# lucidrains/voicebox-pytorch

Hardware: AMD Instinct MI355X
Metric: mel-frames/sec train-step (fwd+bwd+allreduce+clip+Adam) (higher is better)
Workload: dtype f16/bf16 (fp16 forward operands, bf16 backward operands, fp32 accumulate/master); 1 GPU; VoiceBox dim 512 depth 12 heads 16 unconditional, 8x1024 frames per GPU, train; global_batch=8, seq_len=1024, parallelism=dp1

## Files before the change

voicebox-pytorch_amd/csrc/ops.hip:

```cpp
#include "common.hpp"
#include "reduce_roles.hpp"
#include <stdlib.h>

namespace {

VBX_DEV void unpack8_bf16(const uint4 p, float v[8]) {
  const unsigned w[4] = {p.x, p.y, p.z, p.w};
#pragma unroll
  for (int i = 0; i < 4; i++) {
    v[2 * i] = bf16_to_f32((u16)(w[i] & 0xffff));
    v[2 * i + 1] = bf16_to_f32((u16)(w[i] >> 16));
  }
}
VBX_DEV void unpack8_f16(const uint4 p, float v[8]) {
  const unsigned w[4] = {p.x, p.y, p.z, p.w};
#pragma unroll
  for (int i = 0; i < 4; i++) {
    v[2 * i] = f16_to_f32((u16)(w[i] & 0xffff));
    v[2 * i + 1] = f16_to_f32((u16)(w[i] >> 16));
  }
}
VBX_DEV uint4 pack8_h(const float v[8]) {
  return make_uint4(pack_f16x2_sat(v[0], v[1]), pack_f16x2_sat(v[2], v[3]), pack_f16x2_sat(v[4], v[5]), pack_f16x2_sat(v[6], v[7]));
}
// ... 135 lines not shown
    int i0, i1;
    float lam;
    interp_src(n, N, T, i0, i1, lam);
    const float g = bf16_to_f32(demb[row * ld + e]);
    const long id0 = dropped ? null_id : ids[(long)b * T + i0], id1 = dropped ? null_id : ids[(long)b * T + i1];
    if (T == N) {
      atomicAdd(gtable + id0 * E + e, g);
    } else {
      atomicAdd(gtable + id0 * E + e, (1.0f - lam) * g);
      atomicAdd(gtable + id1 * E + e, lam * g);
    }
  }
}

constexpr int CT = 64;
template <int MODE, int KS>
__global__ __launch_bounds__(256) void convpos_fwd_kernel(const float* __restrict__ e, const float* __restrict__ w,
                                                          const float* __restrict__ bias, const uint8_t* __restrict__ mask,
                                                          const float* __restrict__ dxs, float* __restrict__ out, int N,
                                                          int R, int D) {
  extern __shared__ float tile[];
  constexpr int ks = KS;
  const int half = ks / 2;
  const int n0 = blockIdx.x * CT, dbase = blockIdx.y * 64, b = blockIdx.z;
  const int dl = threadIdx.x & 63, ng = threadIdx.x >> 6;
  const int d = dbase + dl;
  const int rows = CT + ks - 1;
  for (int r = ng; r < rows; r += 4) {
    const int n = n0 + r - half;
    float v = 0.f;
    if (n >= 0 && n < N && d < D && (!mask || mask[(long)b * N + n])) v = e[((long)b * N + n) * D + d];
    tile[r * 64 + dl] = v;
  }
  __syncthreads();
  if (d >= D) return;
  float wr[KS];
#pragma unroll
  for (int k = 0; k < ks; k++) wr[k] = w[(long)d * ks + k];
  const float bb = bias[d];
  const int Np = N + R;
  for (int i = 0; i < 16; i++) {
    const int nl = ng * 16 + i, n = n0 + nl;
    if (n >= N) break;
    float acc = bb;
#pragma unroll
    for (int k = 0; k < ks; k++) acc += wr[k] * tile[(nl + k) * 64 + dl];
    const bool m = !mask || mask[(long)b * N + n];
    if (MODE == 0 || MODE == 2) {
      const float ev = e[((long)b * N + n) * D + d];
      out[((long)b * Np + R + n) * D + d] = ev + (m ? (MODE == 2 ? gelu_erf_libm(acc) : gelu_erf(acc)) : 0.f);
    } else {
      const float g = dxs[((long)b * Np + R + n) * D + d];
      out[((long)b * N + n) * D + d] = m ? g * gelu_erf_grad(acc) : 0.f;
    }
  }
}

template <int KS>
__global__ __launch_bounds__(256) void convpos_fwd_segs_kernel(const float* __restrict__ e, const float* __restrict__ w,
                                                               const float* __restrict__ bias, const float* __restrict__ reg,
                                                               const int* __restrict__ seg_start, const int* __restrict__ seg_klen,
                                                               const int* __restrict__ tile_seg, float* __restrict__ out, int R, int D) {
  extern __shared__ float tile[];
  constexpr int ks = KS;
  const int half = ks / 2;
  const int r0 = blockIdx.x * CT, dbase = blockIdx.y * 64;
  const int dl = threadIdx.x & 63, ng = threadIdx.x >> 6;
  const int d = dbase + dl;
// ... 87 lines not shown
    reinterpret_cast<float4*>(dx)[i] = a;
    if (dxb) reinterpret_cast<uint2*>(dxb)[i] = make_uint2(pack_bf16x2(a.x, a.y), pack_bf16x2(a.z, a.w));
  }
}

__global__ void regs_fill_kernel(const float* __restrict__ reg, float* __restrict__ xs, int B, int Np, int R, int D) {
  const long total = (long)B * R * D;
  for (long i = blockIdx.x * (long)blockDim.x + threadIdx.x; i < total; i += (long)gridDim.x * blockDim.x) {
    const int b = (int)(i / ((long)R * D));
    const long rd = i - (long)b * R * D;
    xs[(long)b * Np * D + rd] = reg[rd];
  }
}

template <int KS>
__global__ __launch_bounds__(256) void convpos_bwd_kernel(const float* __restrict__ e, const float* __restrict__ w,
                                                          const uint8_t* __restrict__ mask, const float* __restrict__ dxs,
                                                          const float* __restrict__ dpre, float* __restrict__ de,
                                                          u16* __restrict__ deb, float* __restrict__ wpart, int N, int R,
                                                          int D) {
  extern __shared__ float sm[];
  constexpr int ks = KS;
  static_assert(KS <= 31, "wacc holds the taps in [0, KS) and the bias gradient in [31]");
  const int half = ks / 2;
  const int rows = CT + ks - 1;
  float* te = sm;
  float* tp = sm + rows * 64;
  const int n0 = blockIdx.x * CT, dbase = blockIdx.y * 64, b = blockIdx.z;
  const int dl = threadIdx.x & 63, ng = threadIdx.x >> 6;
  const int d = dbase + dl;
  for (int r = ng; r < rows; r += 4) {
    const int n = n0 + r - half;
    float ve = 0.f, vp = 0.f;
    if (n >= 0 && n < N && d < D) {
      if (!mask || mask[(long)b * N + n]) ve = e[((long)b * N + n) * D + d];
      vp = dpre[((long)b * N + n) * D + d];
    }
    te[r * 64 + dl] = ve;
    tp[r * 64 + dl] = vp;
  }
  __syncthreads();
  float wr[KS], wacc[32];
#pragma unroll
  for (int k = 0; k < 32; k++) wacc[k] = 0.f;
  if (d < D) {
#pragma unroll
    for (int k = 0; k < ks; k++) wr[k] = w[(long)d * ks + k];
    const int Np = N + R;
    for (int i = 0; i < 16; i++) {
      const int nl = ng * 16 + i, n = n0 + nl;
      if (n >= N) break;
      float acc = 0.f;
#pragma unroll
      for (int k = 0; k < ks; k++) acc += wr[k] * tp[(nl + 2 * half - k) * 64 + dl];
      const bool m = !mask || mask[(long)b * N + n];
      const float o = dxs[((long)b * Np + R + n) * D + d] + (m ? acc : 0.f);
      de[((long)b * N + n) * D + d] = o;
      if (deb) deb[((long)b * N + n) * D + d] = f32_to_bf16(o);
      const float dp = tp[(nl + half) * 64 + dl];
#pragma unroll
      for (int k = 0; k < ks; k++) wacc[k] += dp * te[(nl + k) * 64 + dl];
      wacc[31] += dp;
    }
  }
  __syncthreads();
  float* red = sm;
#pragma unroll
  for (int k = 0; k < 32; k++) red[(ng * 64 + dl) * 33 + k] = wacc[k];
  __syncthreads();
  const long chunk = (long)b * gridDim.x + blockIdx.x;
  for (int idx = threadIdx.x; idx < 64 * 32; idx += 256) {
    const int c = idx >> 5, k = idx & 31;
    if (dbase + c < D) {
      const float s = red[(0 * 64 + c) * 33 + k] + red[(1 * 64 + c) * 33 + k] + red[(2 * 64 + c) * 33 + k] +
                      red[(3 * 64 + c) * 33 + k];
      wpart[(chunk * D + dbase + c) * 64 + (k == 31 ? 63 : k)] = s;
    }
  }
}

__global__ void conv_wgrad_finalize_kernel(const float* __restrict__ wpart, int chunks, int D, int ks, float* __restrict__ dw,
                                           float* __restrict__ db) {
  const int idx = blockIdx.x * blockDim.x + threadIdx.x;
  if (idx >= D * 64) return;
  const int d = idx >> 6, k = idx & 63;
  if (k >= ks && k != 63) return;
  float s = 0.f;
  int c = 0;
  for (; c + 4 <= chunks; c += 4) {
    float v[4];
// ... 566 lines not shown
        const float4 v = *reinterpret_cast<const float4*>(reinterpret_cast<const float*>(in) + r * ld + c0);
        acc[0] += v.x; acc[1] += v.y; acc[2] += v.z; acc[3] += v.w;
      }
    }
  }
#pragma unroll
  for (int i = 0; i < W; i++) red[rl][cgi][i] = acc[i];
  __syncthreads();
  if (rl == 0 && c0 < C) {
#pragma unroll
    for (int i = 0; i < W; i++)
      scratch[(long)slab * C + c0 + i] = red[0][cgi][i] + red[1][cgi][i] + red[2][cgi][i] + red[3][cgi][i];
  }
}
__global__ __launch_bounds__(1024) void multi_reduce_kernel(vbx_mr_jobs jobs) {
  __shared__ float red[16][64];
  int j = 0;
#pragma unroll
  for (int i = 1; i < VBX_MR_MAX; i++)
    if (i < jobs.n && (int)blockIdx.x >= jobs.job[i].block0) j = i;
  const vbx_mr_job jb = jobs.job[j];
  mr_role(jb, blockIdx.x - jb.block0, red);
}
__global__ __launch_bounds__(1024) void layer_reduce_kernel(vbx_skr_jobs sj, vbx_mr_jobs mj, int skr_blocks) {
  __shared__ float red[16][64];
  if ((int)blockIdx.x < skr_blocks) {
    int j = 0;
#pragma unroll
    for (int i = 1; i < VBX_SKR_MAX; i++)
      if (i < sj.n && (int)blockIdx.x >= sj.job[i].block0) j = i;
    const vbx_skr_job jb = sj.job[j];
    (void)skr_role(jb, ((long)(blockIdx.x - jb.block0) * 1024 + threadIdx.x) * 4);
    return;
  }
  const int bx = blockIdx.x - skr_blocks;
  int j = 0;
#pragma unroll
  for (int i = 1; i < VBX_MR_MAX; i++)
    if (i < mj.n && bx >= mj.job[i].block0) j = i;
  const vbx_mr_job jb = mj.job[j];
// ... 583 lines not shown

#define VBX_CONV_KS_SWITCH(ks, CALL)                                                                                      \
  switch (ks) {                                                                                                           \
    case 1: CALL(1); break;   case 3: CALL(3); break;   case 5: CALL(5); break;   case 7: CALL(7); break;                 \
    case 9: CALL(9); break;   case 11: CALL(11); break; case 13: CALL(13); break; case 15: CALL(15); break;               \
    case 17: CALL(17); break; case 19: CALL(19); break; case 21: CALL(21); break; case 23: CALL(23); break;               \
    case 25: CALL(25); break; case 27: CALL(27); break; case 29: CALL(29); break; default: CALL(31); break;               \
  }
static inline bool conv_ks_ok(int ks) { return ks >= 1 && ks <= 31 && (ks & 1); }

static int convpos_fwd_impl(const float* e, const float* w, const float* bias, const uint8_t* mask, const float* reg, float* xs, int B,
                            int N, int R, int D, int ksize, bool libm, void* stream) {
  VBX_REQUIRE(e && w && bias && xs, "vbx_convpos_fwd: null pointer");
  VBX_REQUIRE(conv_ks_ok(ksize), "vbx_convpos_fwd: conv_pos_embed_kernel_size must be odd and <= 31 (got %d)", ksize);
  VBX_REQUIRE(R == 0 || reg, "vbx_convpos_fwd: register tokens missing");
  dim3 grid(cdiv(N, CT), cdiv(D, 64), B);
#define VBX_CALL(KS)                                                                                                           \
  if (libm)                                                                                                                    \
    hipLaunchKernelGGL((convpos_fwd_kernel<2, KS>), grid, dim3(256), (CT + KS - 1) * 64 * sizeof(float), ST, e, w, bias, mask, \
                       (const float*)nullptr, xs, N, R, D);                                                                    \
  else                                                                                                                         \
    hipLaunchKernelGGL((convpos_fwd_kernel<0, KS>), grid, dim3(256), (CT + KS - 1) * 64 * sizeof(float), ST, e, w, bias, mask, \
                       (const float*)nullptr, xs, N, R, D)
  VBX_CONV_KS_SWITCH(ksize, VBX_CALL)
#undef VBX_CALL
  VBX_LAUNCH_CHECK();
  if (R > 0) {
    hipLaunchKernelGGL(regs_fill_kernel, dim3(grid_for((long)B * R * D)), dim3(256), 0, ST, reg, xs, B, N + R, R, D);
    VBX_LAUNCH_CHECK();
  }
  return 0;
}

extern "C" int vbx_convpos_fwd(const float* e, const float* w, const float* bias, const uint8_t* mask, const float* reg,
                               float* xs, int B, int N, int R, int D, int ksize, void* stream) {
  return convpos_fwd_impl(e, w, bias, mask, reg, xs, B, N, R, D, ksize, false, stream);
}
extern "C" int vbx_convpos_fwd_libm(const float* e, const float* w, const float* bias, const uint8_t* mask, const float* reg,
                                    float* xs, int B, int N, int R, int D, int ksize, void* stream) {
  return convpos_fwd_impl(e, w, bias, mask, reg, xs, B, N, R, D, ksize, true, stream);
}

extern "C" int vbx_convpos_fwd_segs(const float* e, const float* w, const float* bias, const float* reg, const int* seg_start,
                                    const int* seg_klen, const int* tile_seg, float* xs, int Mp, int R, int D, int ksize, void* stream) {
  VBX_REQUIRE(e && w && bias && xs && seg_start && seg_klen && tile_seg, "vbx_convpos_fwd_segs: null pointer");
// ... 45 lines not shown
  VBX_REQUIRE(dxs && dx && B > 0 && N > 0 && R >= 0 && D % 4 == 0, "vbx_stack_input_bwd: bad args");
  hipLaunchKernelGGL(stack_rows_kernel, dim3(grid_for((long)B * N * D / 4)), dim3(256), 0, ST, dxs, dx, B, N, R, D, 0);
  VBX_LAUNCH_CHECK();
  if (R > 0 && dreg) {
    hipLaunchKernelGGL(dreg_kernel, dim3(cdiv((long)R * D, 256)), dim3(256), 0, ST, dxs, dreg, B, N + R, R, D);
    VBX_LAUNCH_CHECK();
  }
  return 0;
}

extern "C" int vbx_convpos_bwd_chunks(int B, int N) { return B * cdiv(N, CT); }

extern "C" int vbx_convpos_bwd(const float* e, const float* w, const float* bias, const uint8_t* mask, const float* dxs,
                               float* dpre_tmp, float* de, void* de_bf16, float* wpart, float* dreg, int B, int N, int R,
                               int D, int ksize, void* stream) {
  VBX_REQUIRE(e && w && bias && dxs && dpre_tmp && de && wpart, "vbx_convpos_bwd: null pointer");
  VBX_REQUIRE(conv_ks_ok(ksize), "vbx_convpos_bwd: conv_pos_embed_kernel_size must be odd and <= 31 (got %d)", ksize);
  dim3 grid(cdiv(N, CT), cdiv(D, 64), B);
  const int rows = CT + ksize - 1;
#define VBX_CALL(KS)                                                                                                            \
  hipLaunchKernelGGL((convpos_fwd_kernel<1, KS>), grid, dim3(256), rows * 64 * sizeof(float), ST, e, w, bias, mask, dxs, dpre_tmp, \
                     N, R, D)
  VBX_CONV_KS_SWITCH(ksize, VBX_CALL)
#undef VBX_CALL
  VBX_LAUNCH_CHECK();
  size_t lds = (size_t)(2 * rows * 64) * sizeof(float);
  if (lds < (size_t)4 * 64 * 33 * sizeof(float)) lds = (size_t)4 * 64 * 33 * sizeof(float);
  static bool attr[32] = {};
#define VBX_CALL(KS)                                                                                                              \
  {                                                                                                                               \
    if (!attr[KS]) {                                                                                                              \
      (void)hipFuncSetAttribute(reinterpret_cast<const void*>(convpos_bwd_kernel<KS>), hipFuncAttributeMaxDynamicSharedMemorySize, \
                                (int)lds);                                                                                        \
      attr[KS] = true;                                                                                                            \
    }                                                                                                                             \
    hipLaunchKernelGGL(convpos_bwd_kernel<KS>, grid, dim3(256), lds, ST, e, w, mask, dxs, dpre_tmp, de, (u16*)de_bf16, wpart, N,   \
                       R, D);                                                                                                     \
  }
  VBX_CONV_KS_SWITCH(ksize, VBX_CALL)
#undef VBX_CALL
  VBX_LAUNCH_CHECK();
  if (R > 0 && dreg) {
    hipLaunchKernelGGL(dreg_kernel, dim3(cdiv((long)R * D, 256)), dim3(256), 0, ST, dxs, dreg, B, N + R, R, D);
    VBX_LAUNCH_CHECK();
  }
  return 0;
}

extern "C" int vbx_conv_wgrad_finalize(const float* wpart, int chunks, int D, int ksize, float* dw, float* db, void* stream) {
  VBX_REQUIRE(wpart && dw && db && ksize < 63, "vbx_conv_wgrad_finalize: bad args");
  hipLaunchKernelGGL(conv_wgrad_finalize_kernel, dim3(cdiv((long)D * 64, 256)), dim3(256), 0, ST, wpart, chunks, D, ksize, dw, db);
  VBX_LAUNCH_CHECK();
// ... 104 lines not shown
                                    void* stream) {
  VBX_REQUIRE(h1_bf16 && dg_bf16 && dh1_bf16 && scratch && Fp % 64 == 0, "vbx_geglu_bwd_colsum: bad args (Fp must be a multiple of 64)");
  hipLaunchKernelGGL(geglu_bwd_colsum_kernel, dim3(cdiv(Fp / 8, 64), GB_SLABS), dim3(256), 0, ST, (const u16*)h1_bf16,
                     (const u16*)dg_bf16, (u16*)dh1_bf16, (long)M, Fp, scratch);
  VBX_LAUNCH_CHECK();
  return 0;
}

extern "C" int vbx_multi_reduce(const vbx_mr_jobs* jobs, void* stream) {
  VBX_REQUIRE(jobs && jobs->n > 0 && jobs->n <= VBX_MR_MAX, "vbx_multi_reduce: bad job count");
  vbx_mr_jobs j = *jobs;
  int blocks = 0;
  for (int i = 0; i < j.n; i++) {
    VBX_REQUIRE(j.job[i].src && j.job[i].dst && j.job[i].rows > 0 && j.job[i].cols > 0 && j.job[i].batches > 0, "vbx_multi_reduce: bad job %d", i);
    j.job[i].block0 = blocks;
    blocks += j.job[i].batches * cdiv(j.job[i].cols, 64);
  }
  hipLaunchKernelGGL(multi_reduce_kernel, dim3(blocks), dim3(1024), 0, ST, j);
  VBX_LAUNCH_CHECK();
  return 0;
}

extern "C" int vbx_layer_reduce(const vbx_skr_jobs* sjobs, const vbx_mr_jobs* mjobs, void* stream) {
  VBX_REQUIRE(sjobs && sjobs->n > 0 && sjobs->n <= VBX_SKR_MAX && mjobs && mjobs->n > 0 && mjobs->n <= VBX_MR_MAX,
              "vbx_layer_reduce: bad job counts");
  vbx_skr_jobs sj = *sjobs;
  vbx_mr_jobs mj = *mjobs;
  int sb = 0, mb = 0;
  for (int i = 0; i < sj.n; i++) {
    VBX_REQUIRE(sj.job[i].slabs && sj.job[i].dst && sj.job[i].splits >= 1 && sj.job[i].M > 0 && sj.job[i].N > 0 && sj.job[i].N % 4 == 0 &&
                    !sj.job[i].sq,
                "vbx_layer_reduce: bad split-K job %d (N must be a multiple of 4; sq partials are served by vbx_splitk_reduce_multi only)", i);
    sj.job[i].block0 = sb;
    sb += cdiv((long)sj.job[i].M * sj.job[i].N / 4, 1024);
  }
  for (int i = 0; i < mj.n; i++) {
    VBX_REQUIRE(mj.job[i].src && mj.job[i].dst && mj.job[i].rows > 0 && mj.job[i].cols > 0 && mj.job[i].batches > 0,
                "vbx_layer_reduce: bad reduction job %d", i);
    mj.job[i].block0 = mb;
    mb += mj.job[i].batches * cdiv(mj.job[i].cols, 64);
  }
  hipLaunchKernelGGL(layer_reduce_kernel, dim3(sb + mb), dim3(1024), 0, ST, sj, mj, sb);
  VBX_LAUNCH_CHECK();
  return 0;
}

extern "C" int vbx_colsum_scratch_floats(int M, int C) { return CS_SLABS * C; }

extern "C" int vbx_colsum_bf16_partials(const void* in_bf16, int M, int C, int ld, float* scratch, void* stream) {
  VBX_REQUIRE(in_bf16 && scratch && C % 8 == 0 && ld % 8 == 0, "vbx_colsum_bf16_partials: bad args");
  hipLaunchKernelGGL(colsum_stage1<true>, dim3(cdiv(C, 64 * 8), CS_SLABS), dim3(256), 0, ST, in_bf16, (long)M, C, (long)ld, scratch);
  VBX_LAUNCH_CHECK();
  return 0;
}
extern "C" int vbx_colsum_slabs(void) { return CS_SLABS; }
// ... 307 lines not shown
```

voicebox-pytorch_amd/csrc/reduce_roles.hpp:

```cpp
#pragma once
#include "common.hpp"

VBX_DEV float skr_role(const vbx_skr_job& jb, long i4) {
  const long total = (long)jb.M * jb.N;
  if (i4 >= total) return 0.f;
  const int r = (int)(i4 / jb.N), c = (int)(i4 - (long)r * jb.N);
  int dr = r;
  if (jb.rowmap == 1) dr = geglu_row_unmap(r, jb.F);
  if (dr < 0 || dr >= jb.dst_rows) return 0.f;
  float4 s = make_float4(0.f, 0.f, 0.f, 0.f);
  const float* sp = jb.slabs + i4;
  int k = 0;
  for (; k + 4 <= jb.splits; k += 4) {
    float4 v[4];
#pragma unroll
    for (int u = 0; u < 4; u++) v[u] = *reinterpret_cast<const float4*>(sp + (long)(k + u) * total);
#pragma unroll
    for (int u = 0; u < 4; u++) { s.x += v[u].x; s.y += v[u].y; s.z += v[u].z; s.w += v[u].w; }
  }
  for (; k < jb.splits; k++) {
    const float4 v = *reinterpret_cast<const float4*>(sp + (long)k * total);
    s.x += v.x; s.y += v.y; s.z += v.z; s.w += v.w;
  }
  float* o = jb.dst + (long)dr * jb.dst_ld + c;
// ... 9 lines not shown
  return sq;
}

VBX_DEV float block_sum_fixed(float v, float* wsum) {
#pragma unroll
  for (int off = 32; off > 0; off >>= 1) v += __shfl_xor(v, off, 64);
  const int lane = threadIdx.x & 63, wave = threadIdx.x >> 6, nw = (blockDim.x + 63) >> 6;
  if (lane == 0) wsum[wave] = v;
  __syncthreads();
  float t = 0.f;
  if (threadIdx.x == 0)
    for (int w = 0; w < nw; w++) t += wsum[w];
  return t;
}

VBX_DEV void mr_role(const vbx_mr_job& jb, int local, float (*red)[64]) {
  const int cblocks = (jb.cols + 63) >> 6;
  const int b = local / cblocks, cb = local - b * cblocks;
  const int il = threadIdx.x & 63, rl = threadIdx.x >> 6;
  const int c = cb * 64 + il;
  float s = 0.f;
  if (c < jb.cols) {
    const float* p = jb.src + (long)b * jb.src_bstride + c;
    int r = rl;
    for (; r + 48 < jb.rows; r += 64) {
      float v[4];
#pragma unroll
      for (int u = 0; u < 4; u++) v[u] = p[(long)(r + 16 * u) * jb.row_stride];
#pragma unroll
      for (int u = 0; u < 4; u++) s += v[u];
    }
    for (; r < jb.rows; r += 16) s += p[(long)r * jb.row_stride];
  }
  red[rl][il] = s;
  __syncthreads();
  if (rl == 0 && c < jb.cols) {
    float t = 0.f;
#pragma unroll
    for (int k = 0; k < 16; k++) t += red[k][il];
    int dc = c;
    if (jb.rowmap == 1) dc = geglu_row_unmap(c, jb.F);
    if (dc >= 0 && dc < jb.dst_len) jb.dst[(long)b * jb.dst_bstride + dc] = t;
  }
}
```

voicebox-pytorch_amd/csrc/runtime.hip:

```cpp
#include "common.hpp"
#include "wgrad_overlap_plan.hpp"
#include <stdlib.h>
#include <algorithm>
#include <string.h>
#include <string>
#include <vector>

namespace {

inline size_t al256(size_t x) { return (x + 255) & ~(size_t)255; }

struct Carver {
  char* base;
  size_t off = 0;
  explicit Carver(void* b) : base((char*)b) {}
  template <class T>
  T* take(size_t n) {
    off = al256(off);
    T* p = base ? (T*)(base + off) : nullptr;
    off += n * sizeof(T);
    return p;
  }
};

// ... 63 lines not shown
  unsigned *dbr = nullptr, *dbc = nullptr;
  u16 *hg = nullptr, *hgh = nullptr;
  float *glp = nullptr, *glh = nullptr, *gls = nullptr;
};
struct Acts {
  u16 *embed_in, *embed_inh;
  u16 *xcb = nullptr, *dxc = nullptr;
  float *e, *four, *pre, *temb, *ada;
  std::vector<float*> xs;
  std::vector<float*> xc, dskip;
  u16 *cat16 = nullptr, *catb = nullptr;
  float* dcat = nullptr;
  std::vector<ALayer> layer;
  u16 *hf, *hfh;
  float *pred, *per_b;
  float *dx, *dq, *dk, *delta, *slabs, *npart, *npart2, *cpart, *dada, *dtemb, *cs_scratch, *cs_layers, *gpart, *tmp2d, *ada_scratch, *dpre, *de, *wpart,
      *tscratch;
  u16 *dxb, *dg, *dh1, *dhn, *dO, *dqkv, *deb, *dpb, *gl_dp, *demb;
  char* attn_scratch = nullptr;
  u16* dxb2 = nullptr;
  u16* copy[wgrad_overlap::BUF_N][wgrad_overlap::kMaxCopies] = {};
  float* slabs_side = nullptr;
  float* gl_ds;
  size_t slab_floats;
  size_t np_stride = 0, cp_stride = 0, cs_stride = 0, gp_stride = 0;
  size_t bytes;
};

int wgrad_splits(long I, long J, long K) {
  const long tiles = ((I + 127) / 128) * ((J + 127) / 128);
  const long smax = (K + 511) / 512;
// ... 131 lines not shown
    a.dada = c.take<float>((size_t)d.B * d.J);
    a.dtemb = c.take<float>((size_t)d.B * d.Th);
    size_t cs = (size_t)vbx_colsum_scratch_floats((int)d.M, 2 * d.Fp);
    if (cs < (size_t)vbx_geglu_bwd_colsum_slabs() * 2 * d.Fp) cs = (size_t)vbx_geglu_bwd_colsum_slabs() * 2 * d.Fp;
    a.cs_scratch = c.take<float>(cs);
    a.cs_stride = (size_t)vbx_geglu_bwd_colsum_slabs() * 2 * d.Fp;
    a.cs_layers = c.take<float>(a.cs_stride * nreg);
    {
      const int r1 = vbx_qknorm_rope_bwd_gpart_rows(d.B), r2 = d.B * vbx_attn_bwd_fused_tiles(d.Np);
      a.gp_stride = (size_t)2 * (r1 > r2 ? r1 : r2) * d.H * 64;
      a.gpart = c.take<float>(a.gp_stride * nreg);
    }
    a.tmp2d = c.take<float>(2 * d.D);
    a.ada_scratch = c.take<float>(std::max((size_t)vbx_adaln_proj_bwd_scratch_floats(d.B, d.Th, 4 * d.D),
                                           (size_t)vbx_adaln_dtemb_all_scratch_floats(d.L, d.B, d.Th, 4 * d.D)));
    a.dpre = c.take<float>((size_t)d.M0 * d.D);
    a.de = c.take<float>((size_t)d.M0 * d.D);
    a.deb = c.take<u16>((size_t)d.M0 * d.D);
    a.dpb = c.take<u16>((size_t)d.M0 * d.Dop);
    a.wpart = c.take<float>((size_t)vbx_convpos_bwd_chunks(d.B, d.N) * d.D * 64);
    a.tscratch = c.take<float>((size_t)vbx_time_embed_bwd_scratch_floats(d.B, d.D));
    a.gl_ds = m->gateloop ? c.take<float>((size_t)d.M * d.D) : nullptr;
    a.gl_dp = m->gateloop ? c.take<u16>((size_t)d.M * 3 * d.D) : nullptr;
    a.demb = d.E ? c.take<u16>((size_t)d.M0 * d.E) : nullptr;
    if (d.Lc) {
      a.xcb = c.take<u16>((size_t)2 * d.M0 * d.Kp);
      a.dxc = c.take<u16>((size_t)2 * d.M0 * d.D);
    }
    a.dxb2 = c.take<u16>((size_t)d.M * d.D);
    a.attn_scratch = c.take<char>(vbx_attn_bwd_scratch_bytes(d.B, d.H, d.Np));
    if (m->unet) {
// ... 699 lines not shown
  const float* P = m->params;
  float* Gd = m->grads;
  const long* G = m->off;
  WgoGuard guard;
  guard.sd = capturing(st) ? nullptr : wgo_side(false);
  guard.forked = guard.sd != nullptr;
  if (m->stack_only) {
    CK(vbx_stack_input_bwd(a.dx, io->dx, d.R ? Gd + G[VBX_P_REG] : nullptr, d.B, d.N, d.R, d.D, stream));
    if (!m->plain_norm && io->dcond &&
        hipMemcpyAsync(io->dcond, a.dtemb, (size_t)d.B * d.Th * sizeof(float), hipMemcpyDeviceToDevice, st) != hipSuccess) {
      vbx_set_error("vbx_model_backward_embed: copy of d(cond) failed");
      return VBX_EINVAL;
    }
    return guard.done(wgo_sync(guard.sd, st, wgrad_overlap::PT_EMBED_END, -1, d.L));
  }
  CK(vbx_convpos_bwd(a.e, P + G[VBX_P_CONVW], P + G[VBX_P_CONVB], io->attn_mask, a.dx, a.dpre, a.de, a.deb, a.wpart,
                     d.R ? Gd + G[VBX_P_REG] : nullptr, d.B, d.N, d.R, d.D, d.ks, stream));
  CK(vbx_conv_wgrad_finalize(a.wpart, vbx_convpos_bwd_chunks(d.B, d.N), d.D, d.ks, Gd + G[VBX_P_CONVW], Gd + G[VBX_P_CONVB], stream));
  CK(wgrad(a.deb, d.D, a.embed_in, d.Ke, d.D, d.Ke, d.M0, a.slabs, Gd + G[VBX_P_EMBW], d.D, d.Ke, 0, 0, st));
  if (d.E) {
    WPack w;
    carve_wpack(m, w);
    CK(gemm_nn_bf16(a.deb, d.D, w.embb + d.Din, d.Ke, (int)d.M0, d.E, d.D, a.demb, d.E, st));
    if (hipMemsetAsync(Gd + G[VBX_P_CEMB], 0, (size_t)m->V1 * d.E * sizeof(float), st) != hipSuccess) {
      vbx_set_error("vbx_model_backward_embed: memset of the embedding gradient failed");
      return VBX_EINVAL;
    }
    CK(vbx_cond_emb_bwd(a.demb, d.E, io->cond_ids, io->T, io->drop_mask, io->null_id, Gd + G[VBX_P_CEMB], d.B, d.N, d.E, stream));
  }
  if (d.Lc) {
    WPack w;
// ... 152 lines not shown
```

voicebox-pytorch_amd/duration.py:

```python
from random import random

import torch
from torch import nn

from . import _lib
from ._packing import tensors_key
from .align import Aligner, forward_sum_loss, maximum_path
from .masks import mask_from_frac_lengths, prob_mask_like, take_draw
from .model import ConvPositionEmbed, Transformer, exists


def generate_mask_from_repeats(repeats):
    repeats = repeats.int()
    cumsum = repeats.cumsum(dim=-1)
    start = cumsum - repeats
    total = int(cumsum[..., -1].amax().item())
    pos = torch.arange(total, device=repeats.device)
    return (pos >= start[..., None]) & (pos < cumsum[..., None])


class DurationPredictor(nn.Module):
    def __init__(self, *, audio_enc_dec=None, tokenizer=None, num_phoneme_tokens=None, dim_phoneme_emb=512, dim=512, depth=10,
                 dim_head=64, heads=8, ff_mult=4, ff_dropout=0., conv_pos_embed_kernel_size=31, conv_pos_embed_groups=None,
                 attn_dropout=0, attn_flash=False, attn_qk_norm=True, use_gateloop_layers=False, p_drop_prob=0.2,
# ... 276 lines not shown
        ctx.latent = L
        ctx.set_materialize_grads(False)
        return x, emb

    @staticmethod
    def backward(ctx, gx, gemb):
        ids, am8, packed_b, e, cw32, cb32, we, lcb = ctx.saved_tensors
        B, n, E, D, ks, V = ctx.dims
        M, dev, st = B * n, ids.device, _lib.current_stream()
        L = ctx.latent
        if gx is None and gemb is None:
            return (None,) * (14 if L else 12)
        dwe = dbe = dcw = dcb = dpk = dpw = dpb = None
        if gx is not None:
            chunks = _lib.lib().vbx_convpos_bwd_chunks(B, n)
            dpre = torch.empty(M, D, dtype=torch.float32, device=dev)
            de = torch.empty(M, D, dtype=torch.float32, device=dev)
            deb = torch.empty(M, D, dtype=torch.bfloat16, device=dev)
            wpart = torch.zeros(chunks, D, 64, dtype=torch.float32, device=dev)
            _lib.call("vbx_convpos_bwd", e, cw32, cb32, am8, gx.to(torch.float32).contiguous(), dpre, de, deb, wpart, None, B, n, 0, D,
                      ks, st)
            dcw = torch.empty(cw32.shape, dtype=torch.float32, device=dev)
            dcb = torch.empty(D, dtype=torch.float32, device=dev)
            _lib.call("vbx_conv_wgrad_finalize", wpart, chunks, D, ks, dcw, dcb, st)
            dbe = torch.empty(D, dtype=torch.float32, device=dev)
            scratch = torch.empty(_lib.lib().vbx_colsum_scratch_floats(M, D), dtype=torch.float32, device=dev)
            _lib.call("vbx_colsum_f32", de, M, D, D, dbe, scratch, st)
            splits = max(1, min(8, M // 256))
            slabs = torch.empty(splits, D, E + D, dtype=torch.float32, device=dev)
            _gemm(_lib.VBX_GEMM_TN, _lib.VBX_EPI_SPLITK, D, E + D, M, deb, D, packed_b, E + D, slabs, E + D, splits=splits)
            dwe = torch.empty(D, E + D, dtype=torch.float32, device=dev)
            _lib.call("vbx_splitk_reduce", slabs, splits, D, E + D, dwe, D, E + D, E + D, 0, 0, 0, st)
            web = we.detach().to(torch.bfloat16).contiguous() if (ctx.needs_input_grad[7] or L) else None
            if ctx.needs_input_grad[7]:
                dpk = torch.empty(M, E, dtype=torch.float32, device=dev)
# ... 46 lines not shown
```

Baseline: 984,500 mel-frames/s.

## Fuse conv-pos backward recompute into one kernel and widen channel tiles

The conv positional-embedding backward no longer runs a separate kernel that writes the GELU-gradient pre-activation to a global dpre buffer. The single backward kernel now recomputes the conv with halo rows and keeps dpre in LDS, using 512 threads and 128-channel tiles with vectorised float4 tile loads. The forward kernel also fills the register-token rows itself, removing one launch. The multi-row reduction is reworked so each block covers 256 columns with deeper unrolling. The trade-offs are halo recompute, more LDS and register pressure, and explicit FMA-contraction control to keep numerics matching.

```diff
diff --git a/voicebox-pytorch_amd/csrc/ops.hip b/voicebox-pytorch_amd/csrc/ops.hip
--- a/voicebox-pytorch_amd/csrc/ops.hip
+++ b/voicebox-pytorch_amd/csrc/ops.hip
@@ -173,44 +173,121 @@
 }
 
 constexpr int CT = 64;
-template <int MODE, int KS>
+constexpr int CCH = 128;
+
+template <int ROWS, int NT, bool MASKED>
+VBX_DEV void conv_tile_load(const float* __restrict__ src, const uint8_t* __restrict__ mrow, float* tile, int* flag, int n1, int N, int D,
+                            int dbase) {
+  constexpr int RPP = NT / 32, NIT = (ROWS + RPP - 1) / RPP;
+  const int c = dbase + (threadIdx.x & 31) * 4, rr = threadIdx.x >> 5;
+  const bool vec = (D & 3) == 0 && (reinterpret_cast<size_t>(src) & 15) == 0;
+  float4 v[NIT];
+  bool keep[NIT];
+#pragma unroll
+  for (int it = 0; it < NIT; it++) {
+    const int r = rr + it * RPP, n = n1 + r;
+    const bool in = r < ROWS && n >= 0 && n < N;
+    v[it] = make_float4(0.f, 0.f, 0.f, 0.f);
+    keep[it] = in;
+    if (in) {
+      const float* p = src + (long)n * D + c;
+      if (vec) {
+        if (c < D) v[it] = *reinterpret_cast<const float4*>(p);
+      } else {
+        if (c < D) v[it].x = p[0];
+        if (c + 1 < D) v[it].y = p[1];
+        if (c + 2 < D) v[it].z = p[2];
+        if (c + 3 < D) v[it].w = p[3];
+      }
+      if (mrow) keep[it] = mrow[n] != 0;
+    }
+  }
+#pragma unroll
+  for (int it = 0; it < NIT; it++) {
+    const int r = rr + it * RPP;
+    if (r < ROWS) {
+      const bool z = MASKED && !keep[it];
+      *reinterpret_cast<float4*>(tile + r * CCH + (threadIdx.x & 31) * 4) = z ? make_float4(0.f, 0.f, 0.f, 0.f) : v[it];
+      if ((threadIdx.x & 31) == 0) flag[r] = keep[it] ? 1 : 0;
+    }
+  }
+}
+template <int NX, bool SEL>
+VBX_DEV void conv_window(const float* tile, const int* flag, int r0, int ch, float (&x)[NX]) {
+#pragma unroll
+  for (int j = 0; j < NX; j++) {
+    const float v = tile[(r0 + j) * CCH + ch];
+    x[j] = SEL ? (flag[r0 + j] ? v : 0.f) : v;
+  }
+}
+template <int KS, int NOUT>
+VBX_DEV void conv_chain(const float (&wr)[KS], const float (&x)[NOUT + KS - 1], float bb, float (&acc)[NOUT]) {
+#pragma unroll
+  for (int i = 0; i < NOUT; i++) {
+    float a = bb;
+#pragma unroll
+    for (int k = 0; k < KS; k++) a = __builtin_fmaf(wr[k], x[i + k], a);
+    acc[i] = a;
+  }
+}
+
+VBX_DEV float mul_then_add(float a, float b, float c) {
+#pragma clang fp contract(off)
+  const float p = a * b;
+  return c + p;
+}
+
+template <bool LIBM, int KS>
 __global__ __launch_bounds__(256) void convpos_fwd_kernel(const float* __restrict__ e, const float* __restrict__ w,
                                                           const float* __restrict__ bias, const uint8_t* __restrict__ mask,
-                                                          const float* __restrict__ dxs, float* __restrict__ out, int N,
-                                                          int R, int D) {
-  extern __shared__ float tile[];
-  constexpr int ks = KS;
-  const int half = ks / 2;
-  const int n0 = blockIdx.x * CT, dbase = blockIdx.y * 64, b = blockIdx.z;
-  const int dl = threadIdx.x & 63, ng = threadIdx.x >> 6;
-  const int d = dbase + dl;
-  const int rows = CT + ks - 1;
-  for (int r = ng; r < rows; r += 4) {
-    const int n = n0 + r - half;
-    float v = 0.f;
-    if (n >= 0 && n < N && d < D && (!mask || mask[(long)b * N + n])) v = e[((long)b * N + n) * D + d];
-    tile[r * 64 + dl] = v;
-  }
+                                                          const float* __restrict__ reg, float* __restrict__ out, int N, int R,
+                                                          int D) {
+  extern __shared__ float sm[];
+  constexpr int half = KS / 2, rows = CT + KS - 1;
+  float* tile = sm;
+  int* flag = reinterpret_cast<int*>(sm + rows * CCH);
+  const int n0 = blockIdx.x * CT, dbase = blockIdx.y * CCH, b = blockIdx.z;
+  const int Np = N + R;
+  if (blockIdx.x == 0 && R > 0) {
+    const bool vec = (D & 3) == 0 && ((reinterpret_cast<size_t>(reg) | reinterpret_cast<size_t>(out)) & 15) == 0;
+    for (int idx = threadIdx.x; idx < R * 32; idx += 256) {
+      const int r = idx >> 5, c = dbase + (idx & 31) * 4;
+      const float* s = reg + (long)r * D + c;
+      float* o = out + ((long)b * Np + r) * D + c;
+      if (vec) {
+        if (c < D) *reinterpret_cast<float4*>(o) = *reinterpret_cast<const float4*>(s);
+      } else {
+        for (int q = 0; q < 4; q++)
+          if (c + q < D) o[q] = s[q];
+      }
+    }
+  }
+  conv_tile_load<rows, 256, false>(e + (long)b * N * D, mask ? mask + (long)b * N : nullptr, tile, flag, n0 - half, N, D, dbase);
   __syncthreads();
+  const int ch = threadIdx.x & (CCH - 1), ng = threadIdx.x >> 7;
+  const int d = dbase + ch;
   if (d >= D) return;
   float wr[KS];
 #pragma unroll
-  for (int k = 0; k < ks; k++) wr[k] = w[(long)d * ks + k];
+  for (int k = 0; k < KS; k++) wr[k] = w[(long)d * KS + k];
   const float bb = bias[d];
-  const int Np = N + R;
-  for (int i = 0; i < 16; i++) {
-    const int nl = ng * 16 + i, n = n0 + nl;
-    if (n >= N) break;
-    float acc = bb;
-#pragma unroll
-    for (int k = 0; k < ks; k++) acc += wr[k] * tile[(nl + k) * 64 + dl];
-    const bool m = !mask || mask[(long)b * N + n];
-    if (MODE == 0 || MODE == 2) {
-      const float ev = e[((long)b * N + n) * D + d];
-      out[((long)b * Np + R + n) * D + d] = ev + (m ? (MODE == 2 ? gelu_erf_libm(acc) : gelu_erf(acc)) : 0.f);
-    } else {
-      const float g = dxs[((long)b * Np + R + n) * D + d];
-      out[((long)b * N + n) * D + d] = m ? g * gelu_erf_grad(acc) : 0.f;
+  for (int sub = 0; sub < 2; sub++) {
+    const int base = ng * 32 + sub * 16;
+    if (n0 + base >= N) break;
+    float x[16 + KS - 1], acc[16];
+    conv_window<16 + KS - 1, true>(tile, flag, base, ch, x);
+    conv_chain<KS, 16>(wr, x, bb, acc);
+#pragma unroll
+    for (int i = 0; i < 16; i++) {
+      const int nl = base + i, n = n0 + nl;
+      if (n < N) {
+        const float ev = tile[(nl + half) * CCH + ch];
+        const float gl = flag[nl + half] ? (LIBM ? gelu_erf_libm(acc[i]) : gelu_erf(acc[i])) : 0.f;
+        {
+#pragma clang fp contract(off)
+          out[((long)b * Np + R + n) * D + d] = ev + gl;
+        }
+      }
     }
   }
 }
@@ -328,66 +405,94 @@
 }
 
 template <int KS>
-__global__ __launch_bounds__(256) void convpos_bwd_kernel(const float* __restrict__ e, const float* __restrict__ w,
-                                                          const uint8_t* __restrict__ mask, const float* __restrict__ dxs,
-                                                          const float* __restrict__ dpre, float* __restrict__ de,
-                                                          u16* __restrict__ deb, float* __restrict__ wpart, int N, int R,
-                                                          int D) {
+__global__ __launch_bounds__(512) void convpos_bwd_kernel(const float* __restrict__ e, const float* __restrict__ w,
+                                                          const float* __restrict__ bias, const uint8_t* __restrict__ mask,
+                                                          const float* __restrict__ dxs, float* __restrict__ de,
+                                                          u16* __restrict__ deb, float* __restrict__ wpart, int N, int R, int D) {
   extern __shared__ float sm[];
-  constexpr int ks = KS;
   static_assert(KS <= 31, "wacc holds the taps in [0, KS) and the bias gradient in [31]");
-  const int half = ks / 2;
-  const int rows = CT + ks - 1;
+  constexpr int half = KS / 2, RE = CT + 4 * half, RP = CT + 2 * half, HQ = (half + 1) / 2, NW = 16 + KS - 1;
   float* te = sm;
-  float* tp = sm + rows * 64;
-  const int n0 = blockIdx.x * CT, dbase = blockIdx.y * 64, b = blockIdx.z;
-  const int dl = threadIdx.x & 63, ng = threadIdx.x >> 6;
-  const int d = dbase + dl;
-  for (int r = ng; r < rows; r += 4) {
-    const int n = n0 + r - half;
-    float ve = 0.f, vp = 0.f;
-    if (n >= 0 && n < N && d < D) {
-      if (!mask || mask[(long)b * N + n]) ve = e[((long)b * N + n) * D + d];
-      vp = dpre[((long)b * N + n) * D + d];
-    }
-    te[r * 64 + dl] = ve;
-    tp[r * 64 + dl] = vp;
-  }
+  float* tp = sm + RE * CCH;
+  int* flag = reinterpret_cast<int*>(tp + RP * CCH);
+  const int n0 = blockIdx.x * CT, dbase = blockIdx.y * CCH, b = blockIdx.z;
+  const int ch = threadIdx.x & (CCH - 1), ng = threadIdx.x >> 7;
+  const int d = dbase + ch, Np = N + R;
+  const bool dok = d < D;
+  const float* gsrc = dxs + ((long)b * Np + R) * D + d;
+  const int hrow = ng == 0 ? 0 : ng == 1 ? half - HQ : ng == 2 ? CT + half : CT + 2 * half - HQ;
+  float g[16], gh[HQ > 0 ? HQ : 1];
+#pragma unroll
+  for (int i = 0; i < 16; i++) {
+    const int n = n0 + 16 * ng + i;
+    g[i] = dok && n < N ? gsrc[(long)n * D] : 0.f;
+  }
+#pragma unroll
+  for (int i = 0; i < HQ; i++) {
+    const int n = n0 - half + hrow + i;
+    gh[i] = dok && n >= 0 && n < N ? gsrc[(long)n * D] : 0.f;
+  }
+  conv_tile_load<RE, 512, true>(e + (long)b * N * D, mask ? mask + (long)b * N : nullptr, te, flag, n0 - 2 * half, N, D, dbase);
   __syncthreads();
-  float wr[KS], wacc[32];
+  float wr[KS];
+#pragma unroll
+  for (int k = 0; k < KS; k++) wr[k] = dok ? w[(long)d * KS + k] : 0.f;
+  const float bb = dok ? bias[d] : 0.f;
+  {
+    float x[NW], acc[16];
+    conv_window<NW, false>(te, flag, 16 * ng + half, ch, x);
+    conv_chain<KS, 16>(wr, x, bb, acc);
+#pragma unroll
+    for (int i = 0; i < 16; i++)
+      tp[(16 * ng + half + i) * CCH + ch] = flag[16 * ng + 2 * half + i] ? g[i] * gelu_erf_grad(acc[i]) : 0.f;
+  }
+  if constexpr (HQ > 0) {
+    float x[HQ + KS - 1], acc[HQ];
+    conv_window<HQ + KS - 1, false>(te, flag, hrow, ch, x);
+    conv_chain<KS, HQ>(wr, x, bb, acc);
+#pragma unroll
+    for (int i = 0; i < HQ; i++) tp[(hrow + i) * CCH + ch] = flag[hrow + half + i] ? gh[i] * gelu_erf_grad(acc[i]) : 0.f;
+  }
+  __syncthreads();
+  float wacc[32];
 #pragma unroll
   for (int k = 0; k < 32; k++) wacc[k] = 0.f;
-  if (d < D) {
-#pragma unroll
-    for (int k = 0; k < ks; k++) wr[k] = w[(long)d * ks + k];
-    const int Np = N + R;
+  {
+    float xp[NW], xe[NW];
+    conv_window<NW, false>(tp, flag, 16 * ng, ch, xp);
+    conv_window<NW, false>(te, flag, 16 * ng + half, ch, xe);
+#pragma unroll
     for (int i = 0; i < 16; i++) {
-      const int nl = ng * 16 + i, n = n0 + nl;
-      if (n >= N) break;
-      float acc = 0.f;
-#pragma unroll
-      for (int k = 0; k < ks; k++) acc += wr[k] * tp[(nl + 2 * half - k) * 64 + dl];
-      const bool m = !mask || mask[(long)b * N + n];
-      const float o = dxs[((long)b * Np + R + n) * D + d] + (m ? acc : 0.f);
-      de[((long)b * N + n) * D + d] = o;
-      if (deb) deb[((long)b * N + n) * D + d] = f32_to_bf16(o);
-      const float dp = tp[(nl + half) * 64 + dl];
-#pragma unroll
-      for (int k = 0; k < ks; k++) wacc[k] += dp * te[(nl + k) * 64 + dl];
+      const int nl = 16 * ng + i, n = n0 + nl;
+      float acc = __builtin_fmaf(wr[0], xp[i + 2 * half], 0.f);
+#pragma unroll
+      for (int k = 1; k < KS; k++) {
+        const float xv = xp[i + 2 * half - k];
+        acc = k < KS - 12 ? __builtin_fmaf(wr[k], xv, acc) : mul_then_add(wr[k], xv, acc);
+      }
+      if (dok && n < N) {
+        const float o = g[i] + (flag[nl + 2 * half] ? acc : 0.f);
+        de[((long)b * N + n) * D + d] = o;
+        if (deb) deb[((long)b * N + n) * D + d] = f32_to_bf16(o);
+      }
+      const float dp = xp[i + half];
+#pragma unroll
+      for (int k = 0; k < KS - 1; k++) wacc[k] = __builtin_fmaf(dp, xe[i + k], wacc[k]);
+      wacc[KS - 1] = mul_then_add(dp, xe[i + KS - 1], wacc[KS - 1]);
       wacc[31] += dp;
     }
   }
   __syncthreads();
   float* red = sm;
 #pragma unroll
-  for (int k = 0; k < 32; k++) red[(ng * 64 + dl) * 33 + k] = wacc[k];
+  for (int k = 0; k < 32; k++) red[(ng * CCH + ch) * 33 + k] = wacc[k];
   __syncthreads();
   const long chunk = (long)b * gridDim.x + blockIdx.x;
-  for (int idx = threadIdx.x; idx < 64 * 32; idx += 256) {
+  for (int idx = threadIdx.x; idx < CCH * 32; idx += 512) {
     const int c = idx >> 5, k = idx & 31;
     if (dbase + c < D) {
-      const float s = red[(0 * 64 + c) * 33 + k] + red[(1 * 64 + c) * 33 + k] + red[(2 * 64 + c) * 33 + k] +
-                      red[(3 * 64 + c) * 33 + k];
+      const float s = red[(0 * CCH + c) * 33 + k] + red[(1 * CCH + c) * 33 + k] + red[(2 * CCH + c) * 33 + k] +
+                      red[(3 * CCH + c) * 33 + k];
       wpart[(chunk * D + dbase + c) * 64 + (k == 31 ? 63 : k)] = s;
     }
   }
@@ -984,7 +1089,7 @@
   }
 }
 __global__ __launch_bounds__(1024) void multi_reduce_kernel(vbx_mr_jobs jobs) {
-  __shared__ float red[16][64];
+  __shared__ float red[MR_SUBS][16][64];
   int j = 0;
 #pragma unroll
   for (int i = 1; i < VBX_MR_MAX; i++)
@@ -993,7 +1098,7 @@
   mr_role(jb, blockIdx.x - jb.block0, red);
 }
 __global__ __launch_bounds__(1024) void layer_reduce_kernel(vbx_skr_jobs sj, vbx_mr_jobs mj, int skr_blocks) {
-  __shared__ float red[16][64];
+  __shared__ float red[MR_SUBS][16][64];
   if ((int)blockIdx.x < skr_blocks) {
     int j = 0;
 #pragma unroll
@@ -1607,21 +1712,16 @@
   VBX_REQUIRE(e && w && bias && xs, "vbx_convpos_fwd: null pointer");
   VBX_REQUIRE(conv_ks_ok(ksize), "vbx_convpos_fwd: conv_pos_embed_kernel_size must be odd and <= 31 (got %d)", ksize);
   VBX_REQUIRE(R == 0 || reg, "vbx_convpos_fwd: register tokens missing");
-  dim3 grid(cdiv(N, CT), cdiv(D, 64), B);
-#define VBX_CALL(KS)                                                                                                           \
-  if (libm)                                                                                                                    \
-    hipLaunchKernelGGL((convpos_fwd_kernel<2, KS>), grid, dim3(256), (CT + KS - 1) * 64 * sizeof(float), ST, e, w, bias, mask, \
-                       (const float*)nullptr, xs, N, R, D);                                                                    \
-  else                                                                                                                         \
-    hipLaunchKernelGGL((convpos_fwd_kernel<0, KS>), grid, dim3(256), (CT + KS - 1) * 64 * sizeof(float), ST, e, w, bias, mask, \
-                       (const float*)nullptr, xs, N, R, D)
+  dim3 grid(cdiv(N, CT), cdiv(D, CCH), B);
+#define VBX_CALL(KS)                                                                                                         \
+  {                                                                                                                          \
+    const size_t lds = (size_t)(CT + KS - 1) * (CCH * sizeof(float) + sizeof(int));                                          \
+    if (libm) hipLaunchKernelGGL((convpos_fwd_kernel<true, KS>), grid, dim3(256), lds, ST, e, w, bias, mask, reg, xs, N, R, D); \
+    else hipLaunchKernelGGL((convpos_fwd_kernel<false, KS>), grid, dim3(256), lds, ST, e, w, bias, mask, reg, xs, N, R, D);  \
+  }
   VBX_CONV_KS_SWITCH(ksize, VBX_CALL)
 #undef VBX_CALL
   VBX_LAUNCH_CHECK();
-  if (R > 0) {
-    hipLaunchKernelGGL(regs_fill_kernel, dim3(grid_for((long)B * R * D)), dim3(256), 0, ST, reg, xs, B, N + R, R, D);
-    VBX_LAUNCH_CHECK();
-  }
   return 0;
 }
 
@@ -1697,18 +1797,13 @@
 extern "C" int vbx_convpos_bwd(const float* e, const float* w, const float* bias, const uint8_t* mask, const float* dxs,
                                float* dpre_tmp, float* de, void* de_bf16, float* wpart, float* dreg, int B, int N, int R,
                                int D, int ksize, void* stream) {
-  VBX_REQUIRE(e && w && bias && dxs && dpre_tmp && de && wpart, "vbx_convpos_bwd: null pointer");
+  (void)dpre_tmp;
+  VBX_REQUIRE(e && w && bias && dxs && de && wpart, "vbx_convpos_bwd: null pointer");
   VBX_REQUIRE(conv_ks_ok(ksize), "vbx_convpos_bwd: conv_pos_embed_kernel_size must be odd and <= 31 (got %d)", ksize);
-  dim3 grid(cdiv(N, CT), cdiv(D, 64), B);
-  const int rows = CT + ksize - 1;
-#define VBX_CALL(KS)                                                                                                            \
-  hipLaunchKernelGGL((convpos_fwd_kernel<1, KS>), grid, dim3(256), rows * 64 * sizeof(float), ST, e, w, bias, mask, dxs, dpre_tmp, \
-                     N, R, D)
-  VBX_CONV_KS_SWITCH(ksize, VBX_CALL)
-#undef VBX_CALL
-  VBX_LAUNCH_CHECK();
-  size_t lds = (size_t)(2 * rows * 64) * sizeof(float);
-  if (lds < (size_t)4 * 64 * 33 * sizeof(float)) lds = (size_t)4 * 64 * 33 * sizeof(float);
+  dim3 grid(cdiv(N, CT), cdiv(D, CCH), B);
+  const int half = ksize / 2;
+  size_t lds = (size_t)((CT + 4 * half) * CCH + (CT + 2 * half) * CCH) * sizeof(float) + (size_t)(CT + 4 * half) * sizeof(int);
+  if (lds < (size_t)4 * CCH * 33 * sizeof(float)) lds = (size_t)4 * CCH * 33 * sizeof(float);
   static bool attr[32] = {};
 #define VBX_CALL(KS)                                                                                                              \
   {                                                                                                                               \
@@ -1717,8 +1812,7 @@
                                 (int)lds);                                                                                        \
       attr[KS] = true;                                                                                                            \
     }                                                                                                                             \
-    hipLaunchKernelGGL(convpos_bwd_kernel<KS>, grid, dim3(256), lds, ST, e, w, mask, dxs, dpre_tmp, de, (u16*)de_bf16, wpart, N,   \
-                       R, D);                                                                                                     \
+    hipLaunchKernelGGL(convpos_bwd_kernel<KS>, grid, dim3(512), lds, ST, e, w, bias, mask, dxs, de, (u16*)de_bf16, wpart, N, R, D); \
   }
   VBX_CONV_KS_SWITCH(ksize, VBX_CALL)
 #undef VBX_CALL
@@ -1853,7 +1947,7 @@
   for (int i = 0; i < j.n; i++) {
     VBX_REQUIRE(j.job[i].src && j.job[i].dst && j.job[i].rows > 0 && j.job[i].cols > 0 && j.job[i].batches > 0, "vbx_multi_reduce: bad job %d", i);
     j.job[i].block0 = blocks;
-    blocks += j.job[i].batches * cdiv(j.job[i].cols, 64);
+    blocks += j.job[i].batches * cdiv(j.job[i].cols, MR_COLS);
   }
   hipLaunchKernelGGL(multi_reduce_kernel, dim3(blocks), dim3(1024), 0, ST, j);
   VBX_LAUNCH_CHECK();
@@ -1877,7 +1971,7 @@
     VBX_REQUIRE(mj.job[i].src && mj.job[i].dst && mj.job[i].rows > 0 && mj.job[i].cols > 0 && mj.job[i].batches > 0,
                 "vbx_layer_reduce: bad reduction job %d", i);
     mj.job[i].block0 = mb;
-    mb += mj.job[i].batches * cdiv(mj.job[i].cols, 64);
+    mb += mj.job[i].batches * cdiv(mj.job[i].cols, MR_COLS);
   }
   hipLaunchKernelGGL(layer_reduce_kernel, dim3(sb + mb), dim3(1024), 0, ST, sj, mj, sb);
   VBX_LAUNCH_CHECK();
diff --git a/voicebox-pytorch_amd/csrc/reduce_roles.hpp b/voicebox-pytorch_amd/csrc/reduce_roles.hpp
--- a/voicebox-pytorch_amd/csrc/reduce_roles.hpp
+++ b/voicebox-pytorch_amd/csrc/reduce_roles.hpp
@@ -47,30 +47,44 @@
   return t;
 }
 
-VBX_DEV void mr_role(const vbx_mr_job& jb, int local, float (*red)[64]) {
-  const int cblocks = (jb.cols + 63) >> 6;
+constexpr int MR_SUBS = 4;
+constexpr int MR_COLS = 64 * MR_SUBS;
+template <int U>
+VBX_DEV void mr_rows(const float* p, long row_stride, int& r, int rows, const bool (&ok)[MR_SUBS], float (&s)[MR_SUBS]) {
+  for (; r + 16 * (U - 1) < rows; r += 16 * U) {
+    float v[U][MR_SUBS];
+#pragma unroll
+    for (int u = 0; u < U; u++)
+#pragma unroll
+      for (int q = 0; q < MR_SUBS; q++) v[u][q] = ok[q] ? p[(long)(r + 16 * u) * row_stride + 64 * q] : 0.f;
+#pragma unroll
+    for (int u = 0; u < U; u++)
+#pragma unroll
+      for (int q = 0; q < MR_SUBS; q++) s[q] += v[u][q];
+  }
+}
+VBX_DEV void mr_role(const vbx_mr_job& jb, int local, float (*red)[16][64]) {
+  const int cblocks = (jb.cols + MR_COLS - 1) / MR_COLS;
   const int b = local / cblocks, cb = local - b * cblocks;
   const int il = threadIdx.x & 63, rl = threadIdx.x >> 6;
-  const int c = cb * 64 + il;
-  float s = 0.f;
-  if (c < jb.cols) {
-    const float* p = jb.src + (long)b * jb.src_bstride + c;
-    int r = rl;
-    for (; r + 48 < jb.rows; r += 64) {
-      float v[4];
+  const int c0 = cb * MR_COLS + il;
+  float s[MR_SUBS];
+  bool ok[MR_SUBS];
 #pragma unroll
-      for (int u = 0; u < 4; u++) v[u] = p[(long)(r + 16 * u) * jb.row_stride];
+  for (int q = 0; q < MR_SUBS; q++) { s[q] = 0.f; ok[q] = c0 + 64 * q < jb.cols; }
+  const float* p = jb.src + (long)b * jb.src_bstride + c0;
+  int r = rl;
+  mr_rows<8>(p, jb.row_stride, r, jb.rows, ok, s);
+  mr_rows<4>(p, jb.row_stride, r, jb.rows, ok, s);
+  mr_rows<1>(p, jb.row_stride, r, jb.rows, ok, s);
 #pragma unroll
-      for (int u = 0; u < 4; u++) s += v[u];
-    }
-    for (; r < jb.rows; r += 16) s += p[(long)r * jb.row_stride];
-  }
-  red[rl][il] = s;
+  for (int q = 0; q < MR_SUBS; q++) red[q][rl][il] = s[q];
   __syncthreads();
-  if (rl == 0 && c < jb.cols) {
+  const int c = c0 + 64 * rl;
+  if (rl < MR_SUBS && c < jb.cols) {
     float t = 0.f;
 #pragma unroll
-    for (int k = 0; k < 16; k++) t += red[k][il];
+    for (int k = 0; k < 16; k++) t += red[rl][k][il];
     int dc = c;
     if (jb.rowmap == 1) dc = geglu_row_unmap(c, jb.F);
     if (dc >= 0 && dc < jb.dst_len) jb.dst[(long)b * jb.dst_bstride + dc] = t;
diff --git a/voicebox-pytorch_amd/csrc/runtime.hip b/voicebox-pytorch_amd/csrc/runtime.hip
--- a/voicebox-pytorch_amd/csrc/runtime.hip
+++ b/voicebox-pytorch_amd/csrc/runtime.hip
@@ -101,7 +101,7 @@
   std::vector<ALayer> layer;
   u16 *hf, *hfh;
   float *pred, *per_b;
-  float *dx, *dq, *dk, *delta, *slabs, *npart, *npart2, *cpart, *dada, *dtemb, *cs_scratch, *cs_layers, *gpart, *tmp2d, *ada_scratch, *dpre, *de, *wpart,
+  float *dx, *dq, *dk, *delta, *slabs, *npart, *npart2, *cpart, *dada, *dtemb, *cs_scratch, *cs_layers, *gpart, *tmp2d, *ada_scratch, *de, *wpart,
       *tscratch;
   u16 *dxb, *dg, *dh1, *dhn, *dO, *dqkv, *deb, *dpb, *gl_dp, *demb;
   char* attn_scratch = nullptr;
@@ -263,7 +263,6 @@
     a.tmp2d = c.take<float>(2 * d.D);
     a.ada_scratch = c.take<float>(std::max((size_t)vbx_adaln_proj_bwd_scratch_floats(d.B, d.Th, 4 * d.D),
                                            (size_t)vbx_adaln_dtemb_all_scratch_floats(d.L, d.B, d.Th, 4 * d.D)));
-    a.dpre = c.take<float>((size_t)d.M0 * d.D);
     a.de = c.take<float>((size_t)d.M0 * d.D);
     a.deb = c.take<u16>((size_t)d.M0 * d.D);
     a.dpb = c.take<u16>((size_t)d.M0 * d.Dop);
@@ -993,7 +992,7 @@
     }
     return guard.done(wgo_sync(guard.sd, st, wgrad_overlap::PT_EMBED_END, -1, d.L));
   }
-  CK(vbx_convpos_bwd(a.e, P + G[VBX_P_CONVW], P + G[VBX_P_CONVB], io->attn_mask, a.dx, a.dpre, a.de, a.deb, a.wpart,
+  CK(vbx_convpos_bwd(a.e, P + G[VBX_P_CONVW], P + G[VBX_P_CONVB], io->attn_mask, a.dx, nullptr, a.de, a.deb, a.wpart,
                      d.R ? Gd + G[VBX_P_REG] : nullptr, d.B, d.N, d.R, d.D, d.ks, stream));
   CK(vbx_conv_wgrad_finalize(a.wpart, vbx_convpos_bwd_chunks(d.B, d.N), d.D, d.ks, Gd + G[VBX_P_CONVW], Gd + G[VBX_P_CONVB], stream));
   CK(wgrad(a.deb, d.D, a.embed_in, d.Ke, d.D, d.Ke, d.M0, a.slabs, Gd + G[VBX_P_EMBW], d.D, d.Ke, 0, 0, st));
diff --git a/voicebox-pytorch_amd/duration.py b/voicebox-pytorch_amd/duration.py
--- a/voicebox-pytorch_amd/duration.py
+++ b/voicebox-pytorch_amd/duration.py
@@ -314,11 +314,10 @@
         dwe = dbe = dcw = dcb = dpk = dpw = dpb = None
         if gx is not None:
             chunks = _lib.lib().vbx_convpos_bwd_chunks(B, n)
-            dpre = torch.empty(M, D, dtype=torch.float32, device=dev)
             de = torch.empty(M, D, dtype=torch.float32, device=dev)
             deb = torch.empty(M, D, dtype=torch.bfloat16, device=dev)
             wpart = torch.zeros(chunks, D, 64, dtype=torch.float32, device=dev)
-            _lib.call("vbx_convpos_bwd", e, cw32, cb32, am8, gx.to(torch.float32).contiguous(), dpre, de, deb, wpart, None, B, n, 0, D,
+            _lib.call("vbx_convpos_bwd", e, cw32, cb32, am8, gx.to(torch.float32).contiguous(), None, de, deb, wpart, None, B, n, 0, D,
                       ks, st)
             dcw = torch.empty(cw32.shape, dtype=torch.float32, device=dev)
             dcb = torch.empty(D, dtype=torch.float32, device=dev)
```

Result: no change. 991,600 mel-frames/s (median of 6 runs) (+0.7%).
